# julilili42/hockey-env

Hardware: AMD Instinct MI355X
Metric: env-steps/sec at 65536 arenas per MI355X (BASELINE.json metric) (higher is better)
Workload: dtype f32

## Files before the change

### hockey-env_amd/csrc/hk_body.h

```cpp
#pragma once
#include "hk_geom.h"
#include "hk_kernels.h"

namespace hk {

#define SC g_scene
#ifndef SLDS
#define SLDS g_scene_lds
#endif

constexpr int kIslandC = 4;
constexpr int kToiC = 2;
constexpr int kBigC = kMaxIsland;
constexpr uint32_t kEdgeMask[3] = {(1u << 8) | (1u << 10) | (0xFFu << 11),
                                   (1u << 9) | (1u << 10) | (0xFFu << 19),
                                   0x3FFu};
constexpr uint32_t kSensorMask = (1u << 6) | (1u << 7);
constexpr uint32_t kToiPairs = 0x7FFFFFFu & ~kSensorMask & ~((1u << 8) | (1u << 9) | (1u << 10));
constexpr uint32_t pair_mask_of_scene(bool toi) {
  uint32_t m = 0u;
  for (int p = 0; p < NP; ++p)
    if (toi ? (!g_scene.sensor[p] && g_scene.pbodyA[p] >= 3) : g_scene.sensor[p] != 0) m |= 1u << p;
  return m;
}
static_assert(pair_mask_of_scene(true) == kToiPairs && pair_mask_of_scene(false) == kSensorMask,
              "pair masks follow the compiled scene's pair table");

constexpr int kLdsToi = 0, kLdsSal0 = 27, kLdsCnt = 35, kLdsPerLane = 62;
constexpr int kToiQ = 128, kToiItemWords = 9;
constexpr int kLdsWords = kLdsPerLane * 64 + kToiQ * kToiItemWords;

struct Dyn {
  float px[3], py[3], qs[3], qc[3];
  float cx[3], cy[3], a[3];
  float c0x[3], c0y[3], a0[3], al0[3];
  float vx[3], vy[3], w[3];
  float fx[3], fy[3], tq[3];
  float ld[3], ad[3], sleep[3];
  int awake[3];
};

struct Arena {
  Dyn d;
  uint32_t touch, enabled, toiflag, cisl, bisl;
  int keep_mode, max_t, time, done, winner, has1, has2, vel_ref;
  int force_big;
  int n_toi, overflow, n_big;
#ifdef HK_PHASE_TIMERS
  int dg_vit_isl, dg_vit_toi, dg_pit, dg_toi_calls, dg_nc_max;
#endif
  float *man;
  float *ws;
  int64_t n, a;
  float *lds;
  int lane;
#ifdef HK_TRACE
  float *trace;
#endif
};

#ifdef HK_TRACE
constexpr int kTraceStride = 13 + 24 * 4 + 128;
HK_DEV void trace_point(const Arena &w, int k) {
  if (!w.trace) return;
  float *t = w.trace + 13 + 24 * k;
  for (int b = 0; b < 3; ++b) {
    t[6 * b + 0] = w.d.px[b]; t[6 * b + 1] = w.d.py[b]; t[6 * b + 2] = w.d.a[b];
    t[6 * b + 3] = w.d.vx[b]; t[6 * b + 4] = w.d.vy[b]; t[6 * b + 5] = w.d.w[b];
  }
  t[18] = __int_as_float((int)w.touch);
  t[19] = __int_as_float((int)w.enabled);
  t[20] = __int_as_float(w.d.awake[0] | (w.d.awake[1] << 1) | (w.d.awake[2] << 2));
  t[21] = (float)w.n_toi;
  t[22] = (float)w.n_big;
  t[23] = __int_as_float((int)w.cisl);
}
#define HK_TRACE_POINT(w, k) trace_point(w, k)
#define HK_TRACE_SLOT(w, k, s)                                              \
  do {                                                                      \
    if ((w).trace) {                                                        \
      const float *_src = reinterpret_cast<const float *>(&(s));            \
      for (int _q = 0; _q < 64 && _q < (int)(sizeof(s) / 4); ++_q)          \
// ... 190 lines not shown
```

### hockey-env_amd/csrc/hk_core.h

```cpp
#pragma once
#include <hip/hip_runtime.h>
#include <stdint.h>

#ifndef HK_DEV
#define HK_DEV __device__ __forceinline__
#endif

namespace hk {

constexpr float kPi = 3.14159265359f;
constexpr float kLinearSlop = 0.005f;
constexpr float kPolyRadius = 2.0f * kLinearSlop;
constexpr float kMaxTranslation = 2.0f;
constexpr float kMaxRotation = 0.5f * kPi;
constexpr float kBaumgarte = 0.2f;
constexpr float kToiBaumgarte = 0.75f;
constexpr float kMaxLinearCorrection = 0.2f;
constexpr float kVelocityThreshold = 1.0f;
constexpr float kTimeToSleep = 0.5f;
constexpr float kLinearSleepTol = 0.01f;
constexpr float kAngularSleepTol = 2.0f / 180.0f * kPi;
constexpr int kMaxSubSteps = 8;
constexpr int kMaxPolyVerts = 8;
constexpr int kStaticVerts = 4;
// ... 181 lines not shown
  int n = rem_pio2(x, a, b);
  switch (n & 3) {
    case 0: return kcos(a, b);
    case 1: return -ksin(a, b);
    case 2: return -kcos(a, b);
    default: return ksin(a, b);
  }
}

#if defined(__HIP_DEVICE_COMPILE__)
HK_DEV bool wave_any(bool p) { return __ballot(p) != 0ull; }
#else
HK_DEV bool wave_any(bool p) { return p; }
#endif

HK_DEV uint32_t lane_mask(bool c) {
  uint32_t m = c ? 0xffffffffu : 0u;
#if defined(__HIP_DEVICE_COMPILE__)
  asm volatile("" : "+v"(m));
#else
  asm volatile("" : "+r"(m));
#endif
  return m;
}
HK_DEV float mask_f(float x, uint32_t m) { return __builtin_bit_cast(float, __builtin_bit_cast(uint32_t, x) & m); }

#ifdef HK_ASM_MARKS
#define HK_MARK(x) asm volatile(";HKMARK " #x)
#else
#define HK_MARK(x) ((void)0)
#endif

#ifdef HK_PHASE_TIMERS
struct PhaseT {
  unsigned long long last, acc[16], fam[3];
};
#define HK_FAM_T0() const unsigned long long _ft0 = __builtin_amdgcn_s_memtime()
#define HK_FAM_ADD(T, k) ((T).fam[k] += __builtin_amdgcn_s_memtime() - _ft0)
#define HK_TIC(T, k)                                              \
  do {                                                            \
    unsigned long long _t = __builtin_amdgcn_s_memtime();         \
    (T).acc[k] += _t - (T).last;                                  \
    (T).last = _t;                                                \
  } while (0)
#ifdef HK_T0_SPLIT
#define HK_TIC_SPLIT(T, k) HK_TIC(T, k)
#else
#define HK_TIC_SPLIT(T, k) ((void)0)
#endif
#else
struct PhaseT {};
#define HK_TIC_SPLIT(T, k) ((void)0)
#define HK_TIC(T, k) ((void)0)
#define HK_FAM_T0() ((void)0)
#define HK_FAM_ADD(T, k) ((void)0)
#endif

}
```

### hockey-env_amd/csrc/hk_kernels.hip

```cpp
#include "hk_core.h"

alignas(16) constexpr hk::Scene g_scene =
#include "hk_scene_data.inc"
    ;
__shared__ __align__(16) hk::Scene g_scene_lds;

#include "hk_step.h"

namespace hk {

HK_DEV void wave_count(unsigned long long *ctr, int idx, int pred) {
  const unsigned long long m = __ballot(pred);
  if (m && (threadIdx.x & 63) == (__ffsll((long long)m) - 1)) atomicAdd(&ctr[idx], (unsigned long long)__popcll(m));
}

template <int kBlock>
HK_DEV void copy_scene_to_lds() {
  static_assert(sizeof(Scene) % 4 == 0, "the scene copies as words");
  constexpr int kW = (int)(sizeof(Scene) / 4), kQ = kW / 4, kTrips = (kQ + kBlock - 1) / kBlock;
  const uint4 *src = reinterpret_cast<const uint4 *>(&g_scene);
  uint4 *dst = reinterpret_cast<uint4 *>(&g_scene_lds);
  const int t = (int)threadIdx.x;
  uint4 q[kTrips];
#pragma unroll
// ... 23 lines not shown
  StepIO r = io;
  const int64_t o = (int64_t)k * n;
  r.actions = io.actions ? io.actions + o * 8 : nullptr;
  r.opp_inc = io.opp_inc ? io.opp_inc + o * 2 : nullptr;
  r.obs = io.obs ? io.obs + o * 18 : nullptr;
  r.obs2 = io.obs2 ? io.obs2 + o * 18 : nullptr;
  r.reward = io.reward ? io.reward + o : nullptr;
  r.reward2 = io.reward2 ? io.reward2 + o : nullptr;
  r.done = io.done ? io.done + o : nullptr;
  r.info = io.info ? io.info + o * 4 : nullptr;
  r.info2 = io.info2 ? io.info2 + o * 4 : nullptr;
  r.actions_out = io.actions_out ? io.actions_out + o * 8 : nullptr;
  r.final_obs = io.final_obs ? io.final_obs + o * 18 : nullptr;
  r.policy2 = io.policy2 ? io.policy2 + o : nullptr;
  r.record = io.record ? io.record + o * 16 : nullptr;
  r.debug = (k == nsteps - 1) ? io.debug : nullptr;
  return r;
}

#ifndef HK_STEP_BLOCK
#define HK_STEP_BLOCK 64
#endif
#ifndef HK_STEP_OCC
#define HK_STEP_OCC 1
#endif
template <bool kRollout>
__global__ void __launch_bounds__(64, HK_STEP_OCC) step_kernel(DevState s, KCfg cfg, StepIO io, int nsteps) {
  if (!kRollout) nsteps = 1;
  const int64_t a = (int64_t)blockIdx.x * blockDim.x + threadIdx.x;
  const bool live = a < s.n;
  int done_edge = 0, win1 = 0, win2 = 0, ntoi = 0, ovf = 0, nbig = 0, badp = 0, bada = 0;
  PhaseT T;
#ifdef HK_PHASE_TIMERS
  for (int k = 0; k < 16; ++k) T.acc[k] = 0;
  for (int k = 0; k < 3; ++k) T.fam[k] = 0;
  T.last = __builtin_amdgcn_s_memtime();
#endif
  __shared__ float lds[kLdsWords];
  StepWords m;
  if (live) fetch_words(m, s, cfg, step_io(io, 0, nsteps, s.n), a);
  copy_scene_to_lds<HK_STEP_BLOCK>();
  HK_TIC_SPLIT(T, 13);
  if (live) {
    for (int k = 0; k < nsteps; ++k) {
      LaneOut out;
      const StepIO sio = step_io(io, k, nsteps, s.n);
      if (k > 0) fetch_words(m, s, cfg, sio, a);
      step_lane(s, cfg, sio, a, lds, threadIdx.x & 63, T, out, m);
      done_edge += out.done_edge;
      win1 += out.win1;
      win2 += out.win2;
      ntoi += out.ntoi;
      ovf |= out.ovf;
      nbig += out.nbig;
      badp += out.bad_policy;
      bada += out.bad_action;
    }
  }
  if (io.done_word && a == 0)
    __hip_atomic_store(io.done_word, io.done_seq, __ATOMIC_RELEASE, __HIP_MEMORY_SCOPE_SYSTEM);
  const unsigned long long lanes = __ballot(live);
  if ((threadIdx.x & 63) == 0 && lanes) atomicAdd(&s.counters[0], (unsigned long long)__popcll(lanes) * nsteps);
  if (done_edge > 0) atomicAdd(&s.counters[1], (unsigned long long)done_edge);
  if (win1 > 0) atomicAdd(&s.counters[2], (unsigned long long)win1);
  if (win2 > 0) atomicAdd(&s.counters[3], (unsigned long long)win2);
  if (ntoi > 0) atomicAdd(&s.counters[4], (unsigned long long)ntoi);
  wave_count(s.counters, 5, ovf);
  if (nbig > 0) atomicAdd(&s.counters[6], (unsigned long long)nbig);
  if (badp > 0) atomicAdd(&s.counters[7], (unsigned long long)badp);
  if (bada > 0) atomicAdd(&s.counters[9], (unsigned long long)bada);
#ifdef HK_PHASE_TIMERS
  if ((threadIdx.x & 63) == 0)
    for (int k = 0; k < 8; ++k)
      atomicAdd(&s.counters[8 + k], T.acc[k] + (k == 5 ? T.acc[8] + T.acc[9] + T.acc[10] + T.acc[11] + T.acc[12] : 0ull) +
                                        (k == 0 ? T.acc[13] + T.acc[14] + T.acc[15] : 0ull));
  if (io.debug && live) {
    unsigned long long tot = 0;
    for (int k = 0; k < 16; ++k) {
      tot += T.acc[k];
#ifndef HK_T0_SPLIT
      if (k >= 13) continue;
#endif
      io.debug[a * 24 + 8 + k] = (float)T.acc[k];
    }
    io.debug[a * 24] = (float)tot;
  }
#endif
}

HK_DEV unsigned long long wave_bcast(unsigned long long v) {
  const uint32_t lo = __builtin_amdgcn_readfirstlane((uint32_t)v), hi = __builtin_amdgcn_readfirstlane((uint32_t)(v >> 32));
  return ((unsigned long long)hi << 32) | lo;
}
__global__ void __launch_bounds__(64, 1) host_server_kernel(DevState s, KCfg cfg, StepIO io, HostServer hs) {
  const int lane = (int)threadIdx.x;
  const bool live = lane == 0 && s.n == 1;
  __shared__ float lds[kLdsWords];
  copy_scene_to_lds<64>();
  unsigned long long served = 0ull;
  if (lane == 0) served = __hip_atomic_load(hs.done, __ATOMIC_ACQUIRE, __HIP_MEMORY_SCOPE_SYSTEM);
  served = wave_bcast(served);
  const unsigned long long t0 = wall_clock64();
  unsigned long long t_last = t0;
  for (;;) {
    unsigned long long req = 0ull;
    if (lane == 0) req = __hip_atomic_load(hs.req, __ATOMIC_ACQUIRE, __HIP_MEMORY_SCOPE_SYSTEM);
    req = wave_bcast(req);
    if (req == kServerQuit) break;
    const unsigned long long now = wall_clock64();
    if (req == served) {
      if (now - t_last > hs.idle_ticks || now - t0 > hs.life_ticks) break;
      __builtin_amdgcn_s_sleep(2);
      continue;
    }
    int32_t flags = 0, has_act = 0, has_inc = 0;
    if (lane == 0) {
      flags = hs.args[0];
      has_act = hs.args[1];
// ... 108 lines not shown
```

### hockey-env_amd/csrc/hk_solver.h

```cpp
#pragma once

namespace hk {

#ifdef HK_HOST_DIAG
extern unsigned long long g_hk_host_diag[4];
#define HK_HOST_DIAG_INC(k) (++g_hk_host_diag[k])
#else
#define HK_HOST_DIAG_INC(k) ((void)0)
#endif


struct FSlot {
  int bits;
  float mA, mB, iA, iB, fr;
  float nx, ny;
  float rAx[2], rAy[2], rBx[2], rBy[2], ni[2], ti[2], nm[2], tm[2], bias[2];
  float Kxx, Kxy, Kyy, Nxx, Nxy, Nyy;
  uint32_t sn[4];
};
constexpr int kSlotWords = (int)(sizeof(FSlot) / 4);

HK_DEV int fs_pair(const FSlot &s) { return s.bits & 31; }
HK_DEV int fs_isl(const FSlot &s) { return (s.bits >> 5) & 3; }
HK_DEV int fs_bA(const FSlot &s) { return (s.bits >> 7) & 15; }
HK_DEV int fs_bB(const FSlot &s) { return (s.bits >> 11) & 15; }
HK_DEV int fs_vcount(const FSlot &s) { return (s.bits >> 15) & 3; }
HK_DEV int fs_pcount(const FSlot &s) { return (s.bits >> 17) & 3; }
HK_DEV int fs_type(const FSlot &s) { return (s.bits >> 19) & 3; }

HK_DEV void get_vel_a(const Dyn &B, int b, v2 &v, float &w) {
  v = V(pick_a(B.vx, b, 0.0f), pick_a(B.vy, b, 0.0f));
  w = pick_a(B.w, b, 0.0f);
}
HK_DEV void get_vel_b(const Dyn &B, int b, v2 &v, float &w) {
  v = V(pick_b(B.vx, b), pick_b(B.vy, b));
  w = pick_b(B.w, b);
}
HK_DEV void set_vel_a(Dyn &B, int b, v2 v, float w) {
  place_a(B.vx, b, v.x);
  place_a(B.vy, b, v.y);
  place_a(B.w, b, w);
// ... 18 lines not shown
}
HK_DEV void set_pos_a(Dyn &B, int b, v2 c, float a) {
  place_a(B.cx, b, c.x);
  place_a(B.cy, b, c.y);
  place_a(B.a, b, a);
}
HK_DEV void set_pos_b(Dyn &B, int b, v2 c, float a) {
  place(B.cx, b, c.x);
  place(B.cy, b, c.y);
  place(B.a, b, a);
}

HK_DEV float pair_rA() { return kPolyRadius; }
HK_DEV float pair_rB(int bB) { return bB == B_PK ? SC.fx[F_PK].radius : kPolyRadius; }

struct ManGeo {
  int type, count;
  v2 ln, lp, pt[2];
};
HK_DEV ManGeo man_geo(const Arena &w, int p) {
  const Quad *rec = man_rec(w, SLDS.manslot[p]);
  const Quad q0 = rec[0], q1 = rec[1], q2 = rec[2];
  ManGeo g;
  const int meta = __float_as_int(q0.x);
  g.count = meta & 0xff;
  g.type = meta >> 8;
  g.ln = V(q0.y, q0.z);
  g.lp = V(q0.w, q1.x);
  g.pt[0] = V(q1.y, q1.z);
  g.pt[1] = g.count > 1 ? V(q1.w, q2.x) : V(0.0f, 0.0f);
  return g;
}

HK_DEV void fslot_load(FSlot &s, const Arena &w, int p, int warm, int isl) {
  const int pa = SLDS.pbodyA[p], pb = SLDS.pbodyB[p];
  const Quad *rec = man_rec(w, SLDS.manslot[p]);
  const int meta = __float_as_int(rec[0].x);
  const int count = meta & 0xff, type = meta >> 8;
  s.bits = p | (isl << 5) | (pa << 7) | (pb << 11) | (count << 15) | (count << 17) | (type << 19);
  s.fr = SLDS.friction[p];
  s.mA = inv_mass(pa); s.mB = inv_mass(pb); s.iA = inv_inertia(pa); s.iB = inv_inertia(pb);
  s.Kxx = s.Kxy = s.Kyy = 0.0f;
  s.Nxx = s.Nxy = s.Nyy = 0.0f;
  s.nx = s.ny = 0.0f;
  Quad q3 = Quad{0.0f, 0.0f, 0.0f, 0.0f};
  if (warm) q3 = rec[3];
  const float mni[2] = {q3.x, q3.z}, mti[2] = {q3.y, q3.w};
#pragma unroll
  for (int j = 0; j < 2; ++j) {
    const bool on = j < count;
    s.ni[j] = on && warm ? 1.0f * mni[j] : 0.0f;
    s.ti[j] = on && warm ? 1.0f * mti[j] : 0.0f;
    s.rAx[j] = s.rAy[j] = s.rBx[j] = s.rBy[j] = 0.0f;
    s.nm[j] = s.tm[j] = s.bias[j] = 0.0f;
  }
  s.sn[0] = s.sn[1] = s.sn[2] = s.sn[3] = 0u;
}

HK_DEV void fslot_init_velocity(FSlot &s, const Arena &w) {
  const Dyn &B = w.d;
  const float mA = s.mA, mB = s.mB, iA = s.iA, iB = s.iB;
  const int bA = fs_bA(s), bB = fs_bB(s), p = fs_pair(s);
  const float rAr = pair_rA(), rBr = pair_rB(bB);
  v2 cA, cB, vA, vB;
  float aA, aB, wA, wB;
  get_pos_a(B, bA, cA, aA);
  get_pos_b(B, bB, cB, aB);
  get_vel_a(B, bA, vA, wA);
  get_vel_b(B, bB, vB, wB);
  xform xA, xB;
  if (bA >= 3) {
    xA.q.s = 0.0f;
    xA.q.c = 1.0f;
  } else {
    xA.q = rot_set(aA);
  }
  xB.q = rot_set(aB);
  xA.p = vsub(cA, mul_rv(xA.q, local_center(bA)));
  xB.p = vsub(cB, mul_rv(xB.q, local_center(bB)));
  const ManGeo m = man_geo(w, p);
  v2 normal, pts[2];
  if (m.type == 1) {
    normal = mul_rv(xA.q, m.ln);
    v2 plane = mul_xv(xA, m.lp);
#pragma unroll
    for (int i = 0; i < 2; ++i) {
      v2 clip = mul_xv(xB, m.pt[i]);
      v2 ca = vadd(clip, vs(rAr - dot(vsub(clip, plane), normal), normal));
      v2 cb = vsub(clip, vs(rBr, normal));
      pts[i] = vs(0.5f, vadd(ca, cb));
    }
  } else {
    normal = mul_rv(xB.q, m.ln);
    v2 plane = mul_xv(xB, m.lp);
#pragma unroll
    for (int i = 0; i < 2; ++i) {
      v2 clip = mul_xv(xA, m.pt[i]);
      v2 cb = vadd(clip, vs(rBr - dot(vsub(clip, plane), normal), normal));
      v2 ca = vsub(clip, vs(rAr, normal));
      pts[i] = vs(0.5f, vadd(ca, cb));
    }
    normal = vneg(normal);
  }
  s.nx = normal.x;
  s.ny = normal.y;
  const float re = SLDS.restitution[p];
  const int vcount = fs_vcount(s);
  HK_EV(EV_INIT, 1);
  HK_EV(EV_INIT_PT, vcount);
  HK_EV(EV_INIT_BLOCK, vcount == 2);
#pragma unroll
  for (int j = 0; j < 2; ++j) {
    if (j < vcount) {
// ... 329 lines not shown
```

### hockey-env_amd/csrc/hk_step.h

```cpp
#pragma once
#include "hk_arena.h"
#include "hk_seed.h"

namespace hk {

struct U4 { uint32_t x, y, z, w; };
HK_DEV U4 philox(uint64_t seed, uint32_t c0, uint32_t c1, uint32_t c2, uint32_t c3) {
  uint32_t k0 = (uint32_t)seed, k1 = (uint32_t)(seed >> 32);
  U4 c = {c0, c1, c2, c3};
#pragma unroll
  for (int r = 0; r < 10; ++r) {
    uint32_t hi0 = __umulhi(0xD2511F53u, c.x), lo0 = 0xD2511F53u * c.x;
    uint32_t hi1 = __umulhi(0xCD9E8D57u, c.z), lo1 = 0xCD9E8D57u * c.z;
    U4 n = {hi1 ^ c.y ^ k0, lo1, hi0 ^ c.w ^ k1, lo0};
    c = n;
    k0 += 0x9E3779B9u;
    k1 += 0xBB67AE85u;
  }
  return c;
}
HK_DEV float u01f(uint32_t x) { return (float)(x >> 8) * (1.0f / 16777216.0f); }
HK_DEV double u01d(uint32_t a, uint32_t b) {
  return ((double)(a >> 5) * 67108864.0 + (double)(b >> 6)) / 9007199254740992.0;
}
// ... 69 lines not shown
    const rot q = rot_set(w.d.a[b]);
    w.d.qs[b] = q.s;
    w.d.qc[b] = q.c;
    w.d.c0x[b] = w.d.cx[b];
    w.d.c0y[b] = w.d.cy[b];
    w.d.a0[b] = w.d.a[b];
    w.d.al0[b] = 0.0f;
    w.d.vx[b] = fw[o + FB_VX];
    w.d.vy[b] = fw[o + FB_VY];
    w.d.w[b] = fw[o + FB_W];
    w.d.sleep[b] = fw[o + FB_SLEEP];
    w.d.awake[b] = (awake >> b) & 1;
    w.d.fx[b] = 0.0f;
    w.d.fy[b] = 0.0f;
    w.d.tq[b] = 0.0f;
    w.d.ld[b] = 0.0f;
    w.d.ad[b] = 0.0f;
  }
  w.d.fx[B_PK] = fw[F_PFX];
  w.d.fy[B_PK] = fw[F_PFY];
  w.keep_mode = keep_mode;
  w.vel_ref = vel_ref;
  w.has1 = iw[I_HAS1];
  w.has2 = iw[I_HAS2];
  w.time = iw[I_TIME];
  w.done = iw[I_DONE];
  w.winner = iw[I_WINNER];
  w.max_t = iw[I_MAXT];
  w.n_toi = 0;
  w.overflow = 0;
  w.n_big = 0;
  w.force_big = 0;
#ifdef HK_PHASE_TIMERS
  w.dg_vit_isl = w.dg_vit_toi = w.dg_pit = w.dg_toi_calls = w.dg_nc_max = 0;
#endif
  w.touch = (uint32_t)iw[I_TOUCH];
  w.enabled = (uint32_t)iw[I_ENABLED];
  w.toiflag = w.cisl = w.bisl = 0u;
  w.man = s.man;
  w.ws = s.ws;
  w.n = s.n;
  w.a = a;
  w.lds = lds;
  w.lane = lane;
#ifdef HK_TRACE
  w.trace = nullptr;
#endif
}
HK_DEV void load_arena(Arena &w, const DevState &s, int64_t a, int keep_mode, int vel_ref, float *lds, int lane) {
  float fw[NFF];
  uint32_t pw[NPW];
  int32_t iw[NIF];
#pragma unroll
  for (int k = 0; k < NFF; ++k) fw[k] = F(s, k, a);
  load_ints(s, a, pw, iw);
  unpack_arena(w, fw, iw, a, s, keep_mode, vel_ref, lds, lane);
}

HK_DEV void arena_ints(const Arena &w, int awake, int one, int ep, int step, int32_t (&iw)[NIF]) {
  iw[I_AWAKE] = awake;
  iw[I_HAS1] = w.has1;
  iw[I_HAS2] = w.has2;
  iw[I_TIME] = w.time;
  iw[I_DONE] = w.done;
  iw[I_WINNER] = w.winner;
  iw[I_MAXT] = w.max_t;
  iw[I_TOUCH] = (int)w.touch;
// ... 283 lines not shown
  }
  const int done_edge = !was_done && w.done, winner = w.winner;
  int one_new = m.i[I_ONE], ep_new = m.i[I_EPISODE];
  if (cfg.auto_reset && w.done) {
    int one = m.i[I_ONE];
    if (cfg.mode == 0) one = !one;
    const uint32_t ep = (uint32_t)m.i[I_EPISODE];
    float p6[6];
    int mt;
    device_placement(cfg.seed, cfg.arena_offset + a, ep, cfg.mode, one, p6, mt);
    reset_arena(w, p6, mt);
    one_new = one;
    ep_new = (int)(ep + 1);
    observe(w, o);
  }
  float *stage = lds + kLdsPerLane * 64;
  if (io.obs) store_row<18>(io.obs, a, o, stage, lane);
  if (io.obs2) {
    observe_two(w, o);
    store_row<18>(io.obs2, a, o, stage, lane);
  }
  store_arena_changed(w, s, a, m.f, m.pw, one_new, ep_new, (int)(stepc + 1));
  HK_TIC(T, 12);
  out.done_edge = done_edge;
  out.win1 = done_edge && winner == 1;
  out.win2 = done_edge && winner == -1;
  out.ntoi = w.n_toi;
  out.ovf = w.overflow;
  out.nbig = w.n_big;
  out.bad_policy = bad_policy;
  out.bad_action = m.bad_action;
#ifdef HK_PHASE_TIMERS
  if (io.debug) {
    float *d = io.debug + a * 24;
    d[1] = (float)w.n_toi; d[2] = (float)w.dg_vit_isl; d[3] = (float)w.dg_vit_toi; d[4] = (float)w.dg_pit;
    d[5] = (float)w.dg_toi_calls; d[6] = (float)w.dg_nc_max; d[7] = (float)w.n_big;
    d[21] = (float)T.fam[0]; d[22] = (float)T.fam[1]; d[23] = (float)T.fam[2];
  }
#endif
}


HK_DEV void observe_lane(const DevState &s, const KCfg &cfg, int64_t a, float *obs, float *obs2) {
  Arena w;
  load_arena(w, s, a, cfg.keep_mode, cfg.vel_ref, nullptr, 0);
  float o[18];
  if (obs) {
    observe(w, o);
    for (int k = 0; k < 18; ++k) obs[a * 18 + k] = o[k];
  }
  if (obs2) {
    observe_two(w, o);
    for (int k = 0; k < 18; ++k) obs2[a * 18 + k] = o[k];
  }
}

HK_DEV void info_lane(const DevState &s, const KCfg &cfg, int64_t a, double *info, double *info2, double *reward,
                      double *reward2) {
  Arena w;
  load_arena(w, s, a, cfg.keep_mode, cfg.vel_ref, nullptr, 0);
  double i1[4], i2[4];
  info_side<0>(w, i1);
  info_side<1>(w, i2);
  for (int k = 0; k < 4; ++k) {
    if (info) info[a * 4 + k] = i1[k];
    if (info2) info2[a * 4 + k] = i2[k];
  }
  if (reward) reward[a] = compute_reward(w) + i1[1];
  if (reward2) reward2[a] = -compute_reward(w) + i2[1];
}
// ... 68 lines not shown
```

### hockey-env_amd/csrc/hk_velocity.h

```cpp
#pragma once
#include <type_traits>

namespace hk {

HK_DEV int chunk_end(int it) {
  const int e = it + (it < 24 ? 8 : 32);
  return e < kVelIters ? e : kVelIters;
}
static_assert(kVelIters % 4 == 0, "the snapshot period divides the iteration count");
struct Chunk {
  int it, stop, first;
  bool active;
  template <typename Trip>
  HK_DEV void run(Trip &&trip) {
    for (; it < stop && active; it += 4) trip(it + 3 >= first);
    if (it >= kVelIters) active = false;
  }
};

template <int LO, int HI, int N>
HK_DEV uint32_t snap_step(const uint32_t (&x)[N], uint32_t (&sn)[N]) {
  uint32_t d = 0u;
#pragma unroll
  for (int k = LO; k < HI; ++k) {
// ... 65 lines not shown
  HK_MARK(vone_end);
  return c;
}
HK_DEV void vone_family(FSlot &s, Dyn &B, int &it, bool &active, int first) {
  const bool entered = active;
  const int bA = fs_bA(s), bB = fs_bB(s), vc = fs_vcount(s);
  const bool dynA = bA < 3;
  const uint32_t mA = lane_mask(dynA);
  v2 vA2, vB2;
  float wA, wB;
  get_vel_a(B, bA, vA2, wA);
  get_vel_b(B, bB, vB2, wB);
  f2 vA = F2(vA2), vB = F2(vB2);
  uint32_t sn[10];
#pragma unroll
  for (int k = 0; k < 10; ++k) sn[k] = 0u;
  Chunk c{it, it, first, active};
  while (wave_any(c.active)) {
    c.stop = chunk_end(c.it);
    const bool sa = !wave_any(c.active && dynA);
    const bool p1 = !wave_any(c.active && vc != 1), p2 = !wave_any(c.active && vc != 2);
    pick<1, 0>(sa, [&](auto kSA) {
      pick_points(p1, p2, [&](auto kP) {
        c = vone_chunk<decltype(kSA)::value != 0, decltype(kP)::value>(s, dynA, mA, vA, wA, vB, wB, sn, c);
      });
    });
  }
  it = c.it;
  active = c.active;
  if (entered) {
    if (dynA) set_vel_a(B, bA, V2(vA), wA);
    set_vel_b(B, bB, V2(vB), wB);
  }
}

HK_DEV f2 sel2(bool c, f2 a, f2 b) { return f2{c ? a[0] : b[0], c ? a[1] : b[1]}; }
struct TwoState {
  f2 vA0, vB0, vA1, vB1;
  float wA0, wB0, wA1, wB1;
};
struct TwoLane {
  bool two, sep, s2, tb, dA0, dA1;
  uint32_t mA0, mA1;
  bool a1a0, a1b0, b1a0, b1b0;
};
template <int kP0, int kP1, bool kG>
HK_DEV Chunk vtwo_chunk(FSlot &s0, FSlot &s1, TwoState &t, uint32_t (&sn)[20], const TwoLane L, Chunk c, bool &on0,
                        bool &on1) {
  f2 vA0 = t.vA0, vB0 = t.vB0, vA1 = t.vA1, vB1 = t.vB1;
  float wA0 = t.wA0, wB0 = t.wB0, wA1 = t.wA1, wB1 = t.wB1;
  HK_MARK(vtwo_begin);
  c.run([&](bool compare) {
#pragma unroll
    for (int u = 0; u < 4; ++u) {
      if (!kG || on0) {
        reset_static(vA0, wA0, L.mA0);
        fslot_solve_velocity_p<false, kP0>(s0, vA0, wA0, vB0, wB0);
        vA1 = sel2(L.a1a0, vA0, sel2(L.a1b0, vB0, vA1));
        wA1 = L.a1a0 ? wA0 : (L.a1b0 ? wB0 : wA1);
        vB1 = sel2(L.b1a0, vA0, sel2(L.b1b0, vB0, vB1));
        wB1 = L.b1a0 ? wA0 : (L.b1b0 ? wB0 : wB1);
      }
      if (on1) {
        reset_static(vA1, wA1, L.mA1);
        fslot_solve_velocity_p<false, kP1>(s1, vA1, wA1, vB1, wB1);
        vA0 = sel2(L.a1a0, vA1, sel2(L.b1a0, vB1, vA0));
// ... 396 lines not shown
```

### hockey-env_amd/csrc/hk_world.h

```cpp
#pragma once
#include "hk_collide.h"
#include "hk_solver.h"

namespace hk {

template <typename SL>
HK_DEV bool solve_islands(Arena &w, SL &S, float dt, PhaseT &T) {
  constexpr int MAXS = SlotCap<SL>::value;
  const float h = dt;
  int island_of[3] = {-1, -1, -1};
  int nc = 0, nisl = 0;
  uint32_t inis = 0u;
  const uint32_t live = w.enabled & w.touch & ~kSensorMask;
  const int seed_order[3] = {B_PK, B_P2, B_P1};
#pragma unroll
  for (int si = 0; si < 3; ++si) {
    const int seed = seed_order[si];
    if (island_of[seed] >= 0 || !w.d.awake[seed]) continue;
    const int isl = nisl++;
    int st0 = seed, st1 = 0, st2 = 0, sc = 1;
    island_of[seed] = isl;
    while (sc > 0) {
      const int bi = sc == 3 ? st2 : (sc == 2 ? st1 : st0);
      --sc;
// ... 105 lines not shown
template <typename SL>
HK_DEV void toi_island_solve(Arena &w, SL &S, int minc, uint32_t extra, int nc, int db, float sub_dt, PhaseT &T) {
  uint32_t m = extra;
  S.each(nc, [&](FSlot &s, int i) {
    int p = minc;
    if (i > 0) { p = __ffs(m) - 1; m &= m - 1u; }
    fslot_load(s, w, p, 0, 0);
  });
  for (int it = 0; it < 20; ++it) {
    float minSep = 0.0f;
    S.each(nc, [&](FSlot &s, int i) {
      minSep = fslot_solve_position(s, w, kToiBaumgarte, minSep, man_geo(w, fs_pair(s)));
    });
    if (minSep >= -1.5f * kLinearSlop) break;
  }
  HK_TIC(T, 10);
  place(w.d.c0x, db, pick(w.d.cx, db, 0.0f));
  place(w.d.c0y, db, pick(w.d.cy, db, 0.0f));
  place(w.d.a0, db, pick(w.d.a, db, 0.0f));
  S.each(nc, [&](FSlot &s, int) { fslot_init_velocity(s, w); });
  const int isl_of[3] = {db == 0 ? 0 : -1, db == 1 ? 0 : -1, db == 2 ? 0 : -1};
  const int vit = velocity_iterations(S, w.d, nc, isl_of, T);
  HK_TIC(T, 11);
#ifdef HK_PHASE_TIMERS
  w.dg_vit_toi += vit;
#endif
  (void)vit;
#pragma unroll
  for (int b = 0; b < 3; ++b)
    if (b == db) integrate_one(sub_dt, w.d, b);
  sync_xf(w, db);
}

HK_DEV float toi_pair_sweeps(int p, const Sweep &sA, const Sweep &sB) {
  const Proxy<kStaticVerts, true> pA = make_proxy<kStaticVerts, true>(SLDS.fx[SLDS.pairA[p]]);
  const Proxy<kMaxPolyVerts> pB = make_proxy<kMaxPolyVerts>(SLDS.fx[SLDS.pairB[p]]);
  float beta;
  const int st = time_of_impact(pA, pB, sA, sB, 1.0f, beta);
  return st == TOI_TOUCHING ? fmin2(sB.alpha0 + (1.0f - sB.alpha0) * beta, 1.0f) : 1.0f;
}
HK_DEV float toi_pair(Arena &w, int p) {
#ifdef HK_PHASE_TIMERS
  w.dg_toi_calls++;
#endif
  return toi_pair_sweeps(p, body_sweep(w, SLDS.pbodyA[p]), body_sweep(w, SLDS.pbodyB[p]));
}
HK_DEV void toi_drain(Arena &w, uint32_t &pending, uint32_t &below) {
  while (pending) {
    const int p = __ffs(pending) - 1;
    pending &= pending - 1u;
    float alpha = toi_pair(w, p);
    LDS(w, kLdsToi + p) = alpha;
    below = alpha < 1.0f ? (below | (1u << p)) : (below & ~(1u << p));
  }
}

HK_DEV void toi_drain_wave(Arena &w, uint32_t &pending, uint32_t &below) {
#if defined(__HIP_DEVICE_COMPILE__)
  float *q = w.lds + kLdsPerLane * 64;
  const uint64_t lt = (1ull << w.lane) - 1ull;
  while (wave_any(pending != 0u)) {
    const int cnt = __popc(pending);
    int off = 0, total = 0;
#pragma unroll
    for (int b = 0; b < 5; ++b) {
      const uint64_t m = __ballot((cnt >> b) & 1);
// ... 185 lines not shown
    uint32_t m = 0u;
    {
      CoreBoxes cbe;
      core_boxes(w, cbe);
#pragma unroll
      for (int p = 0; p < NP; ++p) {
        if (!((kToiPairs >> p) & 1u)) continue;
        const uint32_t bit = 1u << p;
        if (!(cand & bit)) continue;
        if (pair_far_collide(w, p, &cbe, SC)) pair_update_far(w, p, SC);
        else m |= bit;
      }
    }
    while (m) {
      const int e = __ffs(m) - 1;
      m &= m - 1u;
      const uint32_t ebit = 1u << e;
      const int other = SLDS.pbodyA[e];
      const Sweep backup = body_sweep(w, other);
      if (!((w.bisl >> other) & 1u)) body_advance(w, other, minAlpha);
      pair_update_near(w, e);
      if (!(w.enabled & ebit) || !(w.touch & ebit)) {
        body_set_sweep(w, other, backup);
        continue;
      }
      w.cisl |= ebit;
      extra |= ebit;
      ++nc;
      w.bisl |= 1u << other;
    }
    HK_TIC(T, 9);
    const float sub_dt = (1.0f - minAlpha) * dt;
    if (nc > kBigC) { w.overflow = 1; nc = kBigC; }
    if (nc <= kToiC && !w.force_big) {
      RegSlots<kToiC> S;
      toi_island_solve(w, S, minc, extra, nc, bB, sub_dt, T);
    } else {
      w.n_big++;
      HbmSlots S{w.ws, w.n, w.a};
      toi_island_solve(w, S, minc, extra, nc, bB, sub_dt, T);
    }
    w.bisl = 0u;
    const uint32_t em = pick(kEdgeMask, bB, 0u);
    w.toiflag &= ~em;
    w.cisl &= ~em;
    redo = em;
  }
}

HK_DEV void world_step(Arena &w, PhaseT &T) {
  const float dt = 0.02f;
  collide(w);
  HK_TIC(T, 1);
  HK_TRACE_POINT(w, 0);
  bool done = false;
  if (!w.force_big) {
    RegSlots<kIslandC> S;
    done = solve_islands(w, S, dt, T);
  }
  if (!done) {
    w.n_big++;
    HbmSlots S{w.ws, w.n, w.a};
    solve_islands(w, S, dt, T);
  }
  HK_TIC(T, 4);
  HK_TRACE_POINT(w, 1);
  solve_toi(w, dt, T);
// ... 8 lines not shown
```

### hockey-env_amd/csrc/hostcheck/hk_hostcheck.cpp

```cpp
#include <hip/hip_runtime.h>

#include <cmath>
#include <cstdint>
#include <cstdlib>
#include <cstring>
#include <vector>

static inline int __float_as_int(float x) { int r; std::memcpy(&r, &x, 4); return r; }
static inline unsigned __float_as_uint(float x) { unsigned r; std::memcpy(&r, &x, 4); return r; }
static inline float __int_as_float(int x) { float r; std::memcpy(&r, &x, 4); return r; }
static inline float __uint_as_float(unsigned x) { float r; std::memcpy(&r, &x, 4); return r; }
static inline int __ffs(unsigned x) { return __builtin_ffs((int)x); }
static inline int __popc(unsigned x) { return __builtin_popcount(x); }
static inline uint32_t __umulhi(uint32_t a, uint32_t b) { return (uint32_t)(((uint64_t)a * b) >> 32); }
static inline int __double2hiint(double d) { uint64_t u; std::memcpy(&u, &d, 8); return (int)(u >> 32); }
static inline double __hiloint2double(int hi, int lo) {
  const uint64_t u = ((uint64_t)(uint32_t)hi << 32) | (uint32_t)lo;
  double d;
  std::memcpy(&d, &u, 8);
  return d;
}

#define HK_HOST_DIAG
#include "../hk_core.h"

constexpr hk::Scene g_scene =
#include "../hk_scene_data.inc"
    ;

#define SLDS g_scene
#include "../hk_step.h"
#include "../hk_arena_copy.h"

unsigned long long hk::g_hk_host_diag[4];
unsigned long long hk::g_hk_flop_ev[hk::EV_N];

using namespace hk;

struct HostCtx {
  int64_t n;
  std::vector<float> f, man, ws;
  std::vector<int32_t> i;
  std::vector<double> phase;
  std::vector<unsigned long long> counters;
  std::vector<float> lds;
  DevState s;
  KCfg cfg;
};

extern "C" {

void *hkh_create(int64_t n, const int *cfg6, uint64_t seed, int64_t arena_offset) {
  HostCtx *c = new HostCtx();
  c->n = n;
  c->f.assign((size_t)NFF * n, 0.0f);
  c->i.assign((size_t)NPW * n, 0);
  c->man.assign((size_t)NSOLID * NMF * n, 0.0f);
  c->phase.assign((size_t)3 * n, 0.0);
  c->counters.assign(16, 0ull);
  c->lds.assign((size_t)kLdsWords, 0.0f);
  c->s.f = c->f.data();
  c->s.i = c->i.data();
  c->s.man = c->man.data();
  c->ws.assign((size_t)kBigC * kSlotWords * n, 0.0f);
  c->s.ws = c->ws.data();
  c->s.phase = c->phase.data();
  c->s.counters = c->counters.data();
// ... 49 lines not shown
  HostCtx *c = (HostCtx *)h;
  for (int64_t a = 0; a < c->n; ++a)
    if (!mask || mask[a]) set_state_lane(c->s, c->cfg, a, st, aux);
}

void hkh_observe(void *h, float *obs, float *obs2) {
  HostCtx *c = (HostCtx *)h;
  for (int64_t a = 0; a < c->n; ++a) observe_lane(c->s, c->cfg, a, obs, obs2);
}

void hkh_phase(void *h, double *out) {
  HostCtx *c = (HostCtx *)h;
  for (int64_t a = 0; a < c->n; ++a)
    for (int r = 0; r < 3; ++r) out[a * 3 + r] = c->phase[(size_t)r * c->n + a];
}

void hkh_raw(void *h, float **f, int32_t **i) {
  HostCtx *c = (HostCtx *)h;
  *f = c->f.data();
  *i = c->i.data();
}

void hkh_flop_events(unsigned long long *out) {
  std::memcpy(out, hk::g_hk_flop_ev, sizeof(hk::g_hk_flop_ev));
  std::memset(hk::g_hk_flop_ev, 0, sizeof(hk::g_hk_flop_ev));
}
int hkh_flop_event_count(void) { return hk::EV_N; }

void hkh_diag(unsigned long long *out4) {
  std::memcpy(out4, hk::g_hk_host_diag, sizeof(hk::g_hk_host_diag));
  std::memset(hk::g_hk_host_diag, 0, sizeof(hk::g_hk_host_diag));
}

constexpr int kCntBadIndex = 8;
static void copy_list(const ArenaView &dst, const int64_t *dst_idx, const ArenaView &src, const int64_t *src_idx,
                      int64_t m, unsigned long long *bad) {
  for (int64_t e = 0; e < m; ++e) {
    int64_t di, si;
    if (copy_entry(dst, dst_idx, src, src_idx, e, di, si))
      copy_arena(dst, di, src, si);
    else
      *bad += 1;
  }
}

int64_t hkh_snapshot_bytes(int64_t m) { return m < 0 ? 0 : blob_layout(m).bytes; }

void hkh_snapshot_layout(int32_t *out5) {
  out5[0] = NFF;
  out5[1] = NPW;
  out5[2] = kPhaseRows;
  out5[3] = NSOLID;
  out5[4] = NMF;
}

int hkh_snapshot(void *h, const int64_t *idx, int64_t m, void *blob) {
  HostCtx *c = (HostCtx *)h;
  if (m < 0 || ((uintptr_t)blob & 15)) return -1;
  copy_list(blob_view(blob, m), nullptr, view_of(c->s), idx, m, &c->counters[kCntBadIndex]);
  return 0;
}

int hkh_restore(void *h, const int64_t *idx, int64_t m, const void *blob, int64_t blob_m, const int64_t *rows) {
  HostCtx *c = (HostCtx *)h;
  if (m < 0 || blob_m < 0 || ((uintptr_t)blob & 15)) return -1;
  copy_list(view_of(c->s), idx, blob_view(const_cast<void *>(blob), blob_m), rows, m, &c->counters[kCntBadIndex]);
// ... 17 lines not shown
```

Measured before the change: 253.5 million.

## Add lean single-contact TOI island solver specialized for static body A

Adds a specialized TOI island path for the case where only one contact pair is involved (nc == 1). It runs position passes and the velocity solver with body A treated as static and only body B's state kept in registers, and it reuses the manifold geometry so it is not reloaded. This is meant to cut register pressure and generic-slot overhead in the common single-contact TOI case. The cost is extra code size and a new divergent branch inside the wavefront, along with new timer and diagnostic slots.

```diff
diff --git a/hockey-env_amd/csrc/hk_body.h b/hockey-env_amd/csrc/hk_body.h
--- a/hockey-env_amd/csrc/hk_body.h
+++ b/hockey-env_amd/csrc/hk_body.h
@@ -48,6 +48,7 @@
   int n_toi, overflow, n_big;
 #ifdef HK_PHASE_TIMERS
   int dg_vit_isl, dg_vit_toi, dg_pit, dg_toi_calls, dg_nc_max;
+  int dg_toi_lean;
 #endif
   float *man;
   float *ws;
diff --git a/hockey-env_amd/csrc/hk_core.h b/hockey-env_amd/csrc/hk_core.h
--- a/hockey-env_amd/csrc/hk_core.h
+++ b/hockey-env_amd/csrc/hk_core.h
@@ -237,8 +237,10 @@
 #endif
 
 #ifdef HK_PHASE_TIMERS
+constexpr int kPhaseSlots = 18;
+constexpr int kTimerDebugWords = 28;
 struct PhaseT {
-  unsigned long long last, acc[16], fam[3];
+  unsigned long long last, acc[kPhaseSlots], fam[3];
 };
 #define HK_FAM_T0() const unsigned long long _ft0 = __builtin_amdgcn_s_memtime()
 #define HK_FAM_ADD(T, k) ((T).fam[k] += __builtin_amdgcn_s_memtime() - _ft0)
diff --git a/hockey-env_amd/csrc/hk_kernels.hip b/hockey-env_amd/csrc/hk_kernels.hip
--- a/hockey-env_amd/csrc/hk_kernels.hip
+++ b/hockey-env_amd/csrc/hk_kernels.hip
@@ -79,7 +79,7 @@
   int done_edge = 0, win1 = 0, win2 = 0, ntoi = 0, ovf = 0, nbig = 0, badp = 0, bada = 0;
   PhaseT T;
 #ifdef HK_PHASE_TIMERS
-  for (int k = 0; k < 16; ++k) T.acc[k] = 0;
+  for (int k = 0; k < kPhaseSlots; ++k) T.acc[k] = 0;
   for (int k = 0; k < 3; ++k) T.fam[k] = 0;
   T.last = __builtin_amdgcn_s_memtime();
 #endif
@@ -119,18 +119,19 @@
 #ifdef HK_PHASE_TIMERS
   if ((threadIdx.x & 63) == 0)
     for (int k = 0; k < 8; ++k)
-      atomicAdd(&s.counters[8 + k], T.acc[k] + (k == 5 ? T.acc[8] + T.acc[9] + T.acc[10] + T.acc[11] + T.acc[12] : 0ull) +
-                                        (k == 0 ? T.acc[13] + T.acc[14] + T.acc[15] : 0ull));
+      atomicAdd(&s.counters[8 + k],
+                T.acc[k] + (k == 5 ? T.acc[8] + T.acc[9] + T.acc[10] + T.acc[11] + T.acc[12] + T.acc[16] + T.acc[17] : 0ull) +
+                    (k == 0 ? T.acc[13] + T.acc[14] + T.acc[15] : 0ull));
   if (io.debug && live) {
     unsigned long long tot = 0;
-    for (int k = 0; k < 16; ++k) {
+    for (int k = 0; k < kPhaseSlots; ++k) {
       tot += T.acc[k];
 #ifndef HK_T0_SPLIT
-      if (k >= 13) continue;
-#endif
-      io.debug[a * 24 + 8 + k] = (float)T.acc[k];
-    }
-    io.debug[a * 24] = (float)tot;
+      if (k >= 13 && k < 16) continue;
+#endif
+      io.debug[a * kTimerDebugWords + 8 + k] = (float)T.acc[k];
+    }
+    io.debug[a * kTimerDebugWords] = (float)tot;
   }
 #endif
 }
diff --git a/hockey-env_amd/csrc/hk_solver.h b/hockey-env_amd/csrc/hk_solver.h
--- a/hockey-env_amd/csrc/hk_solver.h
+++ b/hockey-env_amd/csrc/hk_solver.h
@@ -5,8 +5,11 @@
 #ifdef HK_HOST_DIAG
 extern unsigned long long g_hk_host_diag[4];
 #define HK_HOST_DIAG_INC(k) (++g_hk_host_diag[k])
+extern unsigned long long g_hk_host_toi_lean;
+#define HK_HOST_TOI_LEAN_INC() (++g_hk_host_toi_lean)
 #else
 #define HK_HOST_DIAG_INC(k) ((void)0)
+#define HK_HOST_TOI_LEAN_INC() ((void)0)
 #endif
 
 
@@ -91,11 +94,18 @@
   return g;
 }
 
-HK_DEV void fslot_load(FSlot &s, const Arena &w, int p, int warm, int isl) {
+HK_DEV void fslot_load(FSlot &s, const Arena &w, int p, int warm, int isl, const ManGeo *geo = nullptr) {
   const int pa = SLDS.pbodyA[p], pb = SLDS.pbodyB[p];
   const Quad *rec = man_rec(w, SLDS.manslot[p]);
-  const int meta = __float_as_int(rec[0].x);
-  const int count = meta & 0xff, type = meta >> 8;
+  int count, type;
+  if (geo) {
+    count = geo->count;
+    type = geo->type;
+  } else {
+    const int meta = __float_as_int(rec[0].x);
+    count = meta & 0xff;
+    type = meta >> 8;
+  }
   s.bits = p | (isl << 5) | (pa << 7) | (pb << 11) | (count << 15) | (count << 17) | (type << 19);
   s.fr = SLDS.friction[p];
   s.mA = inv_mass(pa); s.mB = inv_mass(pb); s.iA = inv_inertia(pa); s.iB = inv_inertia(pb);
@@ -116,7 +126,7 @@
   s.sn[0] = s.sn[1] = s.sn[2] = s.sn[3] = 0u;
 }
 
-HK_DEV void fslot_init_velocity(FSlot &s, const Arena &w) {
+HK_DEV void fslot_init_velocity(FSlot &s, const Arena &w, const ManGeo *geo = nullptr) {
   const Dyn &B = w.d;
   const float mA = s.mA, mB = s.mB, iA = s.iA, iB = s.iB;
   const int bA = fs_bA(s), bB = fs_bB(s), p = fs_pair(s);
@@ -137,7 +147,7 @@
   xB.q = rot_set(aB);
   xA.p = vsub(cA, mul_rv(xA.q, local_center(bA)));
   xB.p = vsub(cB, mul_rv(xB.q, local_center(bB)));
-  const ManGeo m = man_geo(w, p);
+  const ManGeo m = geo ? *geo : man_geo(w, p);
   v2 normal, pts[2];
   if (m.type == 1) {
     normal = mul_rv(xA.q, m.ln);
diff --git a/hockey-env_amd/csrc/hk_step.h b/hockey-env_amd/csrc/hk_step.h
--- a/hockey-env_amd/csrc/hk_step.h
+++ b/hockey-env_amd/csrc/hk_step.h
@@ -125,7 +125,7 @@
   w.n_big = 0;
   w.force_big = 0;
 #ifdef HK_PHASE_TIMERS
-  w.dg_vit_isl = w.dg_vit_toi = w.dg_pit = w.dg_toi_calls = w.dg_nc_max = 0;
+  w.dg_vit_isl = w.dg_vit_toi = w.dg_pit = w.dg_toi_calls = w.dg_nc_max = w.dg_toi_lean = 0;
 #endif
   w.touch = (uint32_t)iw[I_TOUCH];
   w.enabled = (uint32_t)iw[I_ENABLED];
@@ -475,10 +475,11 @@
   out.bad_action = m.bad_action;
 #ifdef HK_PHASE_TIMERS
   if (io.debug) {
-    float *d = io.debug + a * 24;
+    float *d = io.debug + a * kTimerDebugWords;
     d[1] = (float)w.n_toi; d[2] = (float)w.dg_vit_isl; d[3] = (float)w.dg_vit_toi; d[4] = (float)w.dg_pit;
     d[5] = (float)w.dg_toi_calls; d[6] = (float)w.dg_nc_max; d[7] = (float)w.n_big;
     d[21] = (float)T.fam[0]; d[22] = (float)T.fam[1]; d[23] = (float)T.fam[2];
+    d[26] = (float)w.dg_toi_lean;
   }
 #endif
 }
diff --git a/hockey-env_amd/csrc/hk_velocity.h b/hockey-env_amd/csrc/hk_velocity.h
--- a/hockey-env_amd/csrc/hk_velocity.h
+++ b/hockey-env_amd/csrc/hk_velocity.h
@@ -121,6 +121,22 @@
     if (dynA) set_vel_a(B, bA, V2(vA), wA);
     set_vel_b(B, bB, V2(vB), wB);
   }
+}
+
+HK_DEV int vone_family_static_a(FSlot &s, f2 &vB, float &wB) {
+  const int vc = fs_vcount(s);
+  f2 vA = f2{0.0f, 0.0f};
+  float wA = 0.0f;
+  uint32_t sn[10];
+#pragma unroll
+  for (int k = 0; k < 10; ++k) sn[k] = 0u;
+  Chunk c{0, 0, 7, true};
+  while (wave_any(c.active)) {
+    c.stop = chunk_end(c.it);
+    const bool p1 = !wave_any(c.active && vc != 1), p2 = !wave_any(c.active && vc != 2);
+    pick_points(p1, p2, [&](auto kP) { c = vone_chunk<true, decltype(kP)::value>(s, false, 0u, vA, wA, vB, wB, sn, c); });
+  }
+  return c.it;
 }
 
 HK_DEV f2 sel2(bool c, f2 a, f2 b) { return f2{c ? a[0] : b[0], c ? a[1] : b[1]}; }
diff --git a/hockey-env_amd/csrc/hk_world.h b/hockey-env_amd/csrc/hk_world.h
--- a/hockey-env_amd/csrc/hk_world.h
+++ b/hockey-env_amd/csrc/hk_world.h
@@ -161,6 +161,110 @@
   sync_xf(w, db);
 }
 
+template <int kType>
+HK_DEV float toi_one_position_pass(const ManGeo &m, int pcount, f2 &cA, f2 &cB, float &aB, f2 lcB, float mB, float iB,
+                                   float rBr) {
+  const float mA = 0.0f, iA = 0.0f, rAr = pair_rA();
+  const f2 lcA = f2{0.0f, 0.0f};
+  const f2 ln = F2(m.ln), lp = F2(m.lp);
+  float minSep = 0.0f;
+  HK_EV(EV_POS_PT, pcount);
+#pragma unroll
+  for (int j = 0; j < 2; ++j) {
+    if (j < pcount) {
+      rot qA, qB;
+      qA.s = 0.0f;
+      qA.c = 1.0f;
+      qB = rot_set(aB);
+      const f2 pA = cA - prv(qA, lcA), pB = cB - prv(qB, lcB);
+      f2 normal, point;
+      float sep;
+      if constexpr (kType == 1) {
+        normal = prv(qA, ln);
+        const f2 plane = prv(qA, lp) + pA;
+        const f2 clip = prv(qB, F2(m.pt[j])) + pB;
+        sep = pdot(clip - plane, normal) - rAr - rBr;
+        point = clip;
+      } else {
+        normal = prv(qB, ln);
+        const f2 plane = prv(qB, lp) + pB;
+        const f2 clip = prv(qA, F2(m.pt[j])) + pA;
+        sep = pdot(clip - plane, normal) - rAr - rBr;
+        point = clip;
+        normal = -normal;
+      }
+      const f2 rA = point - cA, rB = point - cB;
+      minSep = fmin2(minSep, sep);
+      float C = fclamp(kToiBaumgarte * (sep + kLinearSlop), -kMaxLinearCorrection, 0.0f);
+      float rnA = pcrs(rA, normal), rnB = pcrs(rB, normal);
+      float K = mA + mB + iA * rnA * rnA + iB * rnB * rnB;
+      float impulse = K > 0.0f ? -C / K : 0.0f;
+      const f2 P = bc(impulse) * normal;
+      cA = cA - bc(mA) * P;
+      cB = cB + bc(mB) * P;
+      aB += iB * pcrs(rB, P);
+    }
+  }
+  return minSep;
+}
+HK_DEV void toi_island_solve_one(Arena &w, int minc, int bA, int db, float sub_dt, PhaseT &T) {
+  HK_HOST_TOI_LEAN_INC();
+#ifdef HK_PHASE_TIMERS
+  w.dg_toi_lean++;
+#endif
+  HK_MARK(toi_lean_begin);
+  const ManGeo m = man_geo(w, minc);
+  FSlot s;
+  fslot_load(s, w, minc, 0, 0, &m);
+  {
+    const int pcount = fs_pcount(s);
+    const f2 lcB = F2(local_center(db));
+    const float mB = s.mB, iB = s.iB, rBr = pair_rB(db);
+    const f2 cA0 = f2{SLDS.spx[bA], SLDS.spy[bA]};
+    v2 c0;
+    float aB;
+    get_pos_b(w.d, db, c0, aB);
+    f2 cB = F2(c0);
+    const auto passes = [&](auto kType) {
+      for (int it = 0; it < 20; ++it) {
+        f2 cA = cA0;
+        const float minSep = toi_one_position_pass<decltype(kType)::value>(m, pcount, cA, cB, aB, lcB, mB, iB, rBr);
+        if (minSep >= -1.5f * kLinearSlop) break;
+      }
+    };
+    if (m.type == 1) passes(kint<1>{});
+    else passes(kint<2>{});
+    HK_MARK(toi_lean_pos_end);
+    HK_TIC(T, 16);
+    place(w.d.cx, db, cB[0]);
+    place(w.d.cy, db, cB[1]);
+    place(w.d.a, db, aB);
+    place(w.d.c0x, db, cB[0]);
+    place(w.d.c0y, db, cB[1]);
+    place(w.d.a0, db, aB);
+  }
+  fslot_init_velocity(s, w, &m);
+  HK_MARK(toi_lean_vel_begin);
+  v2 vB2;
+  float wB;
+  get_vel_b(w.d, db, vB2, wB);
+  f2 vB = F2(vB2);
+  HK_FAM_T0();
+  const int it = vone_family_static_a(s, vB, wB);
+  HK_FAM_ADD(T, 2);
+  set_vel_b(w.d, db, V2(vB), wB);
+  HK_TIC(T, 17);
+#ifdef HK_PHASE_TIMERS
+  w.dg_vit_toi += it;
+#endif
+  (void)it;
+#pragma unroll
+  for (int b = 0; b < 3; ++b)
+    if (b == db) integrate_one(sub_dt, w.d, b);
+  sync_xf(w, db);
+  HK_MARK(toi_lean_end);
+}
+
 HK_DEV float toi_pair_sweeps(int p, const Sweep &sA, const Sweep &sB) {
   const Proxy<kStaticVerts, true> pA = make_proxy<kStaticVerts, true>(SLDS.fx[SLDS.pairA[p]]);
   const Proxy<kMaxPolyVerts> pB = make_proxy<kMaxPolyVerts>(SLDS.fx[SLDS.pairB[p]]);
@@ -412,7 +516,9 @@
     HK_TIC(T, 9);
     const float sub_dt = (1.0f - minAlpha) * dt;
     if (nc > kBigC) { w.overflow = 1; nc = kBigC; }
-    if (nc <= kToiC && !w.force_big) {
+    if (nc == 1 && !w.force_big) {
+      toi_island_solve_one(w, minc, bA, bB, sub_dt, T);
+    } else if (nc <= kToiC && !w.force_big) {
       RegSlots<kToiC> S;
       toi_island_solve(w, S, minc, extra, nc, bB, sub_dt, T);
     } else {
diff --git a/hockey-env_amd/csrc/hostcheck/hk_hostcheck.cpp b/hockey-env_amd/csrc/hostcheck/hk_hostcheck.cpp
--- a/hockey-env_amd/csrc/hostcheck/hk_hostcheck.cpp
+++ b/hockey-env_amd/csrc/hostcheck/hk_hostcheck.cpp
@@ -33,6 +33,7 @@
 #include "../hk_arena_copy.h"
 
 unsigned long long hk::g_hk_host_diag[4];
+unsigned long long hk::g_hk_host_toi_lean;
 unsigned long long hk::g_hk_flop_ev[hk::EV_N];
 
 using namespace hk;
@@ -148,6 +149,12 @@
   std::memset(hk::g_hk_host_diag, 0, sizeof(hk::g_hk_host_diag));
 }
 
+unsigned long long hkh_toi_lean(void) {
+  const unsigned long long n = hk::g_hk_host_toi_lean;
+  hk::g_hk_host_toi_lean = 0ull;
+  return n;
+}
+
 constexpr int kCntBadIndex = 8;
 static void copy_list(const ArenaView &dst, const int64_t *dst_idx, const ArenaView &src, const int64_t *src_idx,
                       int64_t m, unsigned long long *bad) {
```

Measured after the change: 256.1 million, median of 6. +1.0%, better.
